# henintsoa98/srsRAN_4G

Hardware: AMD Instinct MI355X
Metric: turbo-decoded info Mbps + PDSCH subframes/s, 20 MHz 64QAM, 1/2/4/8 GPU (higher is better)
Workload: dtype int16; 1 GPU; tdec all 188 LTE CB sizes x 1024 CBs, 8 half-its, rm_turbo SB layout; cb_sizes=188, parallelism=cb-sharded x1, tdec16=auto

## Files before the change

srsran_4g_amd/csrc/tdec_api.cpp:

```cpp
#include <hip/hip_runtime.h>

#include <cstdio>
#include <cstdlib>
#include <algorithm>
#include <cstring>
#include <map>
#include <tuple>
#include <mutex>
#include <vector>

#include "../../include/srsran_tdec.h"
#include "stage_copy.h"
#include "dev_buf.h"
#include "devkey.h"
#include "tdec_kernel.h"
#include "tdec8bit_kernel.h"

using namespace srsran_amd;

namespace {

const uint16_t kCbSizes[SRSRAN_NOF_TC_CB_SIZES] = {
    40,   48,   56,   64,   72,   80,   88,   96,   104,  112,  120,  128,  136,  144,  152,  160,  168,  176,  184,
    192,  200,  208,  216,  224,  232,  240,  248,  256,  264,  272,  280,  288,  296,  304,  312,  320,  328,  336,
// ... 678 lines not shown
  const uint32_t len = (layout_sb && c->nsb > 1) ? 3 * (long_cb + 32) + 12 : 3 * long_cb + 12;
  if (in_stride < len) {
    return SRSRAN_ERROR_INVALID_INPUTS;
  }
  const int n_end = nof_iterations > 0 ? (int)nof_iterations : 1;
  return enqueue(c, d_input, in_stride, layout_sb, d_output, nof_cb, 0, n_end, nullptr, (hipStream_t)stream);
}

namespace {
constexpr int kPoolStreams = 4;
struct MultiDesc {
  PinBuf<char> h_stage;
  DevBuf<char> d_stage;
  hipEvent_t copied  = nullptr;
  bool       used    = false;
};

struct StreamPool {
  int         device = -1;
  hipStream_t s[kPoolStreams];
  hipEvent_t  done[kPoolStreams];
  hipEvent_t  fork;
  hipEvent_t  large_done;
  MultiDesc   md[6];
};
std::mutex               g_pool_mu;
std::vector<StreamPool*> g_pools;

int multi_mode()
{
  static const int m = [] {
    const char* e = getenv("SRSRAN_AMD_TDEC_MULTI");
    return !e ? 0 : !strcmp(e, "priority") ? 1 : !strcmp(e, "serial") ? 2 : 0;
  }();
  return m;
}

StreamPool* get_pool()
{
  int dev = 0;
  if (hipGetDevice(&dev) != hipSuccess) {
    return nullptr;
  }
  std::lock_guard<std::mutex> lk(g_pool_mu);
  for (auto* p : g_pools) {
    if (p->device == dev) {
      return p;
// ... 16 lines not shown
  }
  for (auto& m : p->md) {
    if (srsran_amd::ring_event_create(&m.copied) != hipSuccess) {
      return nullptr;
    }
  }
  g_pools.push_back(p);
  return p;
}

uint32_t gen_cut()
{
  static const uint32_t c = [] {
    const char* e = getenv("SRSRAN_AMD_TDEC_GEN_CUT");
    return e ? (uint32_t)atoi(e) : 0u;
  }();
  return c;
}

uint32_t tdec_midcut()
{
  static const uint32_t c = [] {
    const char* e = getenv("SRSRAN_AMD_TDEC_MIDCUT");
    return e ? (uint32_t)atoi(e) : 3072u;
  }();
  return c;
}
bool tdec_gate()
{
  static const bool g = [] {
    const char* e = getenv("SRSRAN_AMD_TDEC_GATE");
    return e ? atoi(e) != 0 : true;
  }();
  return g;
}

double launch_cost(uint32_t K, uint32_t ncb)
{
  const int    nsb   = auto_nsb(K);
  const double chain = nsb > 1 ? 3.0 * (K / nsb) + 160.0 : 3.0 * (K + 3);
  const double waves = (double)ncb * 4 * nsb / 64.0;
  return chain * (1.0 + waves / 1024.0);
}
}

int srsran_tdec_gpu_run_multi(uint32_t              nof_groups,
                              const uint32_t*       long_cb,
                              const int16_t* const* d_input,
                              const uint32_t*       in_stride,
                              int                   layout_sb,
                              uint8_t* const*       d_output,
                              const uint32_t*       nof_cb,
                              uint32_t              nof_iterations,
                              void*                 stream)
{
  if (nof_groups == 0) {
    return SRSRAN_SUCCESS;
// ... 13 lines not shown
    }
    const uint32_t len = (layout_sb && cfg[g]->nsb > 1) ? 3 * (long_cb[g] + 32) + 12 : 3 * long_cb[g] + 12;
    if (in_stride[g] < len) {
      return SRSRAN_ERROR_INVALID_INPUTS;
    }
    order[g] = g;
  }
  std::sort(order.begin(), order.end(), [&](uint32_t a, uint32_t b) {
    return launch_cost(long_cb[a], nof_cb[a]) > launch_cost(long_cb[b], nof_cb[b]);
  });
  StreamPool* p = get_pool();
  if (!p) {
    return SRSRAN_ERROR;
  }
  hipStream_t user = (hipStream_t)stream;
  if (hipEventRecord(p->fork, user) != hipSuccess) {
    return SRSRAN_ERROR;
  }
  for (int i = 0; i < kPoolStreams; i++) {
    hipStreamWaitEvent(p->s[i], p->fork, 0);
  }
  const int n_end = nof_iterations > 0 ? (int)nof_iterations : 1;
  int       ret   = SRSRAN_SUCCESS;
  const int      cls_nsb[6] = {16, 16, 16, 8, 1, 1};
  const int      cls_st[6]  = {0, 0, 1, 2, 3, 3};
  const uint32_t midcut     = tdec_midcut();
  bool           gated      = false;
  bool           mid_run    = false;
  for (int ci = 0; ci < 6 && ret == SRSRAN_SUCCESS; ci++) {
    if (ci == 1 && hipEventRecord(p->large_done, p->s[0]) != hipSuccess) {
      ret = SRSRAN_ERROR;
      break;
    }
    gated = ci >= 2 && mid_run && tdec_gate() && multi_mode() != 2;
    std::vector<uint32_t> gs;
    uint32_t              cls_cb = 0;
    for (uint32_t i = 0; i < nof_groups; i++) {
      if (cfg[order[i]]->nsb == cls_nsb[ci] && nof_cb[order[i]] > 0) {
        gs.push_back(order[i]);
        cls_cb += nof_cb[order[i]];
      }
    }
    if (gs.empty()) {
      continue;
    }
    const int kind = cls_nsb[ci] == 1               ? (cls_cb >= tdec1s_min_cb() ? 2 : 0)
                     : !layout_sb                   ? 0
                     : cls_nsb[ci] == 16            ? tdec16_choice(cls_cb)
                                                    : (cls_cb >= tdec8s_min_cb() ? 2 : 0);
    const uint32_t cut = std::max(tdecs_w8_max_k(), tdecs_w8_fused_max_k());
    if (cls_nsb[ci] == 16 && kind == 2) {
      const uint32_t lo = ci == 0 ? std::max(cut, midcut) : ci == 1 ? cut : 0;
      const uint32_t hi = ci == 0 ? UINT32_MAX : ci == 1 ? std::max(cut, midcut) : cut;
      gs.erase(std::remove_if(gs.begin(), gs.end(),
                              [&](uint32_t g) { return !(cfg[g]->proto.K > lo && cfg[g]->proto.K <= hi); }),
               gs.end());
    } else if (ci == 1 || ci == 2) {
      gs.clear();
    } else if (ci >= 4 && kind == 0 && gen_cut() > 0) {
      const bool small = ci == 5;
      gs.erase(std::remove_if(gs.begin(), gs.end(), [&](uint32_t g) { return (cfg[g]->proto.K <= gen_cut()) != small; }),
               gs.end());
    } else if (ci == 5) {
      gs.clear();
    }
    if (gs.empty()) {
      continue;
    }
    mid_run        = mid_run || ci == 1;
    hipStream_t st = p->s[multi_mode() == 2 ? 0 : cls_st[ci]];
    if (gated && st != p->s[0] && hipStreamWaitEvent(st, p->large_done, 0) != hipSuccess) {
      ret = SRSRAN_ERROR;
      break;
    }
    if (gs.size() == 1) {
      const uint32_t g = gs[0];
      ret = enqueue(cfg[g], d_input[g], in_stride[g], layout_sb, d_output[g], nof_cb[g], 0, n_end, nullptr, st);
      continue;
    }
    const int  nsbc = cls_nsb[ci];
    uint32_t   kmax = 0;
    for (uint32_t g : gs) {
      kmax = std::max(kmax, cfg[g]->proto.K);
    }
    const bool w8  = kind == 2 && nsbc > 1 && kmax <= (nsbc == 16 ? cut : tdecs_w8_max_k());
    const int  cpw  = kind == 2   ? (nsbc == 16 ? tdecs16::cpw() : nsbc == 8 ? tdecs8::cpw() : tdecs1::cpw())
                      : kind == 1 ? tdec16_cpw()
                                  : tdec_cpw(nsbc);
    const size_t   n     = gs.size();
    const size_t   abyte = n * sizeof(TdecArgs);
    const size_t   need  = abyte + n * sizeof(uint32_t);
    MultiDesc&     m     = p->md[ci];
    if (m.used) {
      hipEventSynchronize(m.copied);
    }
    if (need > m.h_stage.cap() || need > m.d_stage.cap()) {
      hipStreamSynchronize(st);
      if (!m.h_stage.reserve(2 * need) || !m.d_stage.reserve(2 * need)) {
        return SRSRAN_ERROR;
      }
    }
    TdecArgs* ha    = reinterpret_cast<TdecArgs*>(m.h_stage.get());
    uint32_t* hf    = reinterpret_cast<uint32_t*>(m.h_stage + abyte);
    uint32_t  nblk  = 0;
    size_t    lds   = 0;
    for (size_t k = 0; k < n; k++) {
      const uint32_t g = gs[k];
      const Config*  c = cfg[g];
      TdecArgs       a = c->proto;
      a.in             = d_input[g];
      a.in_stride      = in_stride[g];
      a.layout_sb      = c->nsb > 1 ? layout_sb : 0;
      a.ncb            = nof_cb[g];
      a.n_start        = 0;
      a.n_end          = n_end;
      a.out            = d_output[g];
      a.tfwd           = c->d_tfwd;
      a.trev           = c->d_trev;
      a.tfwd_nat       = c->d_tfwd_nat;
      a.trev_nat       = c->d_trev_nat;
      a.state          = nullptr;
      ha[k]            = a;
      hf[k]            = nblk;
      nblk += (nof_cb[g] + cpw - 1) / cpw;
      lds = std::max(lds, kind == 2   ? (nsbc == 16  ? (w8 ? tdecs16w8::lds_bytes(a) : tdecs16::lds_bytes(a))
                                         : nsbc == 8 ? (w8 ? tdecs8w8::lds_bytes(a) : tdecs8::lds_bytes(a))
                                                     : tdecs1::lds_bytes(a))
                          : kind == 1 ? tdec16_lds_bytes(a)
                                      : tdec_lds_bytes(c->nsb, a.xyw, a.M));
    }
    if (hipMemcpyAsync(m.d_stage, m.h_stage, need, hipMemcpyHostToDevice, st) != hipSuccess) {
      return SRSRAN_ERROR;
    }
    hipEventRecord(m.copied, st);
    m.used = true;
    const TdecArgs* dg = reinterpret_cast<const TdecArgs*>(m.d_stage.get());
    const uint32_t* df = reinterpret_cast<const uint32_t*>(m.d_stage + abyte);
    if ((kind == 2   ? (nsbc == 16  ? (w8 ? tdecs16w8::multi_launch(dg, df, (int)n, nblk, lds, st)
                                          : tdecs16::multi_launch(dg, df, (int)n, nblk, lds, st))
                        : nsbc == 8 ? (w8 ? tdecs8w8::multi_launch(dg, df, (int)n, nblk, lds, st)
                                          : tdecs8::multi_launch(dg, df, (int)n, nblk, lds, st))
                                    : tdecs1::multi_launch(dg, df, (int)n, nblk, lds, st))
         : kind == 1 ? tdec16_multi_launch(dg, df, (int)n, nblk, lds, st)
                     : tdec_multi_launch(cls_nsb[ci], dg, df, (int)n, nblk, lds, st)) != hipSuccess) {
      ret = SRSRAN_ERROR;
    }
  }
  for (int i = 0; i < kPoolStreams; i++) {
    hipEventRecord(p->done[i], p->s[i]);
    hipStreamWaitEvent(user, p->done[i], 0);
  }
  return ret;
}

#ifdef TDECS_STAMPS
int srsran_tdec_gpu_debug_set_stamps(void* d_buf)
{
  using namespace srsran_amd;
  return tdecs16::set_stamps(d_buf) == hipSuccess && tdecs8::set_stamps(d_buf) == hipSuccess &&
                 tdecs16w8::set_stamps(d_buf) == hipSuccess && tdecs8w8::set_stamps(d_buf) == hipSuccess
             ? SRSRAN_SUCCESS
             : SRSRAN_ERROR;
// ... 117 lines not shown
```

srsran_4g_amd/csrc/tdec_kernel.h:

```cpp
#ifndef SRSRAN_AMD_TDEC_KERNEL_H
#define SRSRAN_AMD_TDEC_KERNEL_H
#include <hip/hip_runtime.h>
#include <stddef.h>
#include <stdint.h>

namespace srsran_amd {

static constexpr int TDEC_W       = 32;
static constexpr int TDEC_OVERLAP = 40;

struct TdecCb {
  const short*   in;
  const uint8_t* skip;
  uint32_t       slot;
  uint32_t       crc_a;
};
static constexpr uint32_t TDEC_PAD_SLOT = 0xffffffffu;
static constexpr uint64_t TDEC_PAIR_SPAN = ((uint64_t)1 << 31) - ((uint64_t)1 << 16);
static constexpr uint32_t TDEC_GROUP     = 8;

struct TdecArgs {
  const short*    in;
  uint32_t        in_stride;
  int             layout_sb;
// ... 33 lines not shown
bool       tdec16_eligible(int nsb, const TdecArgs& a);
bool       tdec16_pays(uint32_t ncb);
void       tdec16_set_min_cb(uint32_t n);
uint32_t   tdec16_min_cb();
hipError_t tdec16_launch(const TdecArgs& a, hipStream_t stream);
hipError_t tdec16_multi_launch(const TdecArgs* d_groups, const uint32_t* d_first, int ngroups, uint32_t nblocks,
                               size_t lds, hipStream_t stream);
size_t     tdec16_lds_bytes(const TdecArgs& a);
int        tdec16_cpw();
#define SRSRAN_TDECS_API(ns)                                                                               \
  namespace ns {                                                                                           \
  hipError_t launch(const TdecArgs& a, hipStream_t stream);                                                \
  hipError_t multi_launch(const TdecArgs* d_groups, const uint32_t* d_first, int ngroups, uint32_t nblocks, \
                          size_t lds, hipStream_t stream);                                                 \
  size_t     lds_bytes(const TdecArgs& a);                                                                 \
  int        cpw();                                                                                        \
  }
SRSRAN_TDECS_API(tdecs16)
SRSRAN_TDECS_API(tdecs8)
SRSRAN_TDECS_API(tdecs16w8)
SRSRAN_TDECS_API(tdecs8w8)
SRSRAN_TDECS_API(tdecs1)
#undef SRSRAN_TDECS_API
#ifdef TDECS_STAMPS
namespace tdecs16 { hipError_t set_stamps(void* d_buf); }
namespace tdecs8 { hipError_t set_stamps(void* d_buf); }
namespace tdecs16w8 { hipError_t set_stamps(void* d_buf); }
namespace tdecs8w8 { hipError_t set_stamps(void* d_buf); }
#endif
bool       tdec8s_eligible(int nsb, const TdecArgs& a);
bool       tdec1s_eligible(int nsb, const TdecArgs& a);
void       tdecs_set_w8_max_k(uint32_t k);
void       tdecs_set_w8_fused_max_k(uint32_t k);
uint32_t   tdecs_w8_fused_max_k();
uint32_t   tdecs_w8_max_k();
void       tdec8s_set_min_cb(uint32_t n);
uint32_t   tdec8s_min_cb();
void       tdec1s_set_min_cb(uint32_t n);
uint32_t   tdec1s_min_cb();
void       tdec16s_set_min_cb(uint32_t n);
uint32_t   tdec16s_min_cb();
int        tdec16_choice(uint32_t ncb);
size_t     tdec_lds_bytes(int nsb, int xyw, int M);
void crc24_xpow_table(uint32_t poly, uint32_t* out, int nm);

int tdec_sch_enqueue(uint32_t      K,
// ... 18 lines not shown
```

srsran_4g_amd/csrc/tdecs_kernel.hip:

```cpp
#include <hip/hip_runtime.h>
#include <stdint.h>

#include "crc24_dev.h"
#include "stage_timing.h"
#include "tdec_kernel.h"

#ifndef TDECS_NSB
#define TDECS_NSB 16
#endif
#ifndef TDECS_W
#define TDECS_W 16
#endif
#if TDECS_NSB == 16 && TDECS_W == 16
#define TDECS_NS tdecs16
#define TDECS_K(n) tdec16s_##n
#define TDECS_NAME "tdec16s_"
#elif TDECS_NSB == 8 && TDECS_W == 16
#define TDECS_NS tdecs8
#define TDECS_K(n) tdec8s_##n
#define TDECS_NAME "tdec8s_"
#elif TDECS_NSB == 16 && TDECS_W == 8
#define TDECS_NS tdecs16w8
#define TDECS_K(n) tdec16sw8_##n
#define TDECS_NAME "tdec16sw8_"
#elif TDECS_NSB == 8 && TDECS_W == 8
#define TDECS_NS tdecs8w8
#define TDECS_K(n) tdec8sw8_##n
#define TDECS_NAME "tdec8sw8_"
#else
#error "TDECS_NSB must be 16 or 8, TDECS_W 16 or 8"
#endif

namespace srsran_amd {
namespace TDECS_NS {
namespace {

typedef short v2s __attribute__((ext_vector_type(2)));

constexpr int   W    = TDECS_W;
constexpr int   OVL  = TDEC_OVERLAP;
constexpr int   NTR  = (OVL + W - 1) / W;
constexpr int   NSB  = TDECS_NSB;
constexpr short NEG  = -10000;
constexpr int   CPWG = 64 / NSB;
constexpr int   ROWB = 2 * NSB;

#ifdef TDECS_STAMPS
__device__ unsigned long long* g_stamps = nullptr;
#define TDECS_STAMP(k)                                                                               \
  do {                                                                                               \
    if ((threadIdx.x & 63) == 0 && g_stamps && (k) < 64) {                                          \
      g_stamps[((size_t)blockIdx.x * (blockDim.x >> 6) + (threadIdx.x >> 6)) * 64 + (k)] = clock64(); \
    }                                                                                                \
  } while (0)
// ... 91 lines not shown
#pragma unroll
  for (int t = 2; t >= 0; t--) {
    const short x = xt[t], y = yt[t], xy = (short)(x + y);
    short       n[8];
    n[0] = max(o[0], (short)(o[4] + xy));
    n[1] = max((short)(o[0] + xy), o[4]);
    n[2] = max((short)(o[1] + x), (short)(o[5] + y));
    n[3] = max((short)(o[1] + y), (short)(o[5] + x));
    n[4] = max((short)(o[2] + y), (short)(o[6] + x));
    n[5] = max((short)(o[2] + x), (short)(o[6] + y));
    n[6] = max((short)(o[3] + xy), o[7]);
    n[7] = max(o[3], (short)(o[7] + xy));
#pragma unroll
    for (int i = 0; i < 8; i++) {
      o[i] = n[i];
    }
  }
  return St{v2s{o[0], o[4]}, v2s{o[7], o[3]}, v2s{o[2], o[6]}, v2s{o[5], o[1]}};
}

struct Geo {
  int s_dw, ck_dw, bits_dw, cb_dw;
};
__host__ __device__ __forceinline__ Geo geo(int K, int Ls, int M, bool slot)
{
  Geo g;
  g.s_dw    = (NSB * Ls + 1) / 2;
  g.ck_dw   = M * NSB * 4;
  g.bits_dw = slot ? (NSB * Ls + 31) / 32 + 1 : (K / 8 + 3) / 4;
  g.cb_dw   = g.s_dw + g.ck_dw + g.bits_dw + 2;
  return g;
}

struct Raw {
  uint32_t a[W];
  uint16_t slot[W];
  uint32_t b[W];
};

typedef short __attribute__((address_space(3)))* lshort;
typedef __amdgpu_buffer_rsrc_t                   rsrc_t;
__device__ __forceinline__ uint32_t ldb(rsrc_t r, uint32_t voff, uint32_t soff, int imm)
{
  return __builtin_amdgcn_raw_buffer_load_b16(r, voff + imm, soff, 0);
}
__device__ __forceinline__ rsrc_t make_rsrc(const void* p, uint32_t bytes)
{
  const size_t   u  = (size_t)p;
  const uint32_t lo = __builtin_amdgcn_readfirstlane((uint32_t)u);
  const uint32_t hi = __builtin_amdgcn_readfirstlane((uint32_t)(u >> 32));
  return __builtin_amdgcn_make_buffer_rsrc((void*)(((size_t)hi << 32) | lo), 0,
                                           (int)__builtin_amdgcn_readfirstlane(bytes), 0x00020000);
}

struct Lane {
  int       s, K, L, Ls, M, KP;
  uint32_t  magicLs;
  rsrc_t    rin;
  uint32_t  voff;
  rsrc_t    rtf;
  lshort    S;
  lshort    Ssb;
  uint4*    CK;
  uint32_t* BITS;
};

__device__ __forceinline__ void ck_put(const Lane& c, int m, const St& p)
{
  c.CK[m * NSB + c.s] = make_uint4(v2u(p.a), v2u(p.b), v2u(p.c), v2u(p.d));
}
__device__ __forceinline__ St ck_get(const Lane& c, int m)
{
  const uint4 v = c.CK[m * NSB + c.s];
  return St{u2v(v.x), u2v(v.y), u2v(v.z), u2v(v.w)};
}

template <bool D2>
__device__ __forceinline__ void issue(const Lane& c, Raw& r, int t0)
{
  const uint32_t soff = (uint32_t)ROWB * (uint32_t)t0;
  const uint32_t poff = soff + (D2 ? 4u : 2u) * (uint32_t)c.KP;
#ifdef TDECS_FAKELOAD
#pragma unroll
  for (int i = 0; i < W; i++) {
    r.a[i]    = (soff + i) & 0xff;
    r.slot[i] = (uint16_t)((c.s * 37 + t0 + i) & 511);
    r.b[i] = (poff + 3 * i) & 0xff;
  }
#else
#pragma unroll
  for (int i = 0; i < W; i++) {
    if (D2) {
      r.slot[i] = (uint16_t)ldb(c.rtf, 2u * (uint32_t)c.s, soff, ROWB * i);
    } else {
      r.a[i] = ldb(c.rin, c.voff, soff, ROWB * i);
    }
    r.b[i] = ldb(c.rin, c.voff, poff, ROWB * i);
  }
#endif
}

__device__ __forceinline__ uint32_t pin(uint32_t v)
{
  asm volatile("" : "+v"(v));
  return v;
}

__device__ __forceinline__ void set_nat(const Lane& c, int n, short o)
{
  atomicOr(&c.BITS[n >> 5], (uint32_t)(o > 0) << (((n >> 3) & 3) * 8 + 7 - (n & 7)));
}

template <bool D2, int BITS>
__device__ __forceinline__ uint32_t emit(const Lane& c, int k, short o, uint32_t aux, uint32_t xw)
{
  if (D2) {
    const lshort p = (lshort)(size_t)aux;
    *p             = (short)(o - (short)(xw & 0xffffu));
    if (BITS == 2) {
      const uint32_t slot = (uint32_t)(p - c.S);
      atomicOr(&c.BITS[slot >> 5], (uint32_t)(o > 0) << (slot & 31));
    } else if (BITS == 1) {
      const int slot = (int)(p - c.S);
      const int sb   = (int)__umulhi((uint32_t)slot, c.magicLs);
      set_nat(c, slot - sb * (c.Ls - c.L), o);
    }
    return 0;
  }
// ... 10 lines not shown
    const uint32_t pos = (uint32_t)(c.s * c.Ls + t0);
    const uint64_t v   = (uint64_t)wbits << (pos & 31);
    atomicOr(&c.BITS[pos >> 5], (uint32_t)v);
    if ((uint32_t)(v >> 32)) {
      atomicOr(&c.BITS[(pos >> 5) + 1], (uint32_t)(v >> 32));
    }
  }
}

__device__ __forceinline__ uint32_t nat_byte(const uint32_t* bits, int L, int Ls, uint32_t magicL, int b)
{
  const int      n0  = 8 * b;
  const int      j   = (int)__umulhi((uint32_t)n0, magicL);
  const int      cnt = (j + 1) * L - n0;
  const uint32_t s0  = (uint32_t)(n0 + j * (Ls - L));
  const uint64_t v   = (uint64_t)bits[s0 >> 5] | (uint64_t)bits[(s0 >> 5) + 1] << 32;
  uint32_t       x   = (uint32_t)(v >> (s0 & 31)) & 0x1ffu;
  if (cnt < 8) {
    x = (x & ((1u << cnt) - 1u)) | ((x >> (cnt + Ls - L)) << cnt);
  }
  return __builtin_bitreverse32(x & 0xffu) >> 24;
}

template <bool D2, int BITS, bool FULL>
__device__ __forceinline__ St alpha_llr_window(const Lane& c, St P, int t0, St Pb, const uint32_t* xw,
                                               const uint32_t* aux)
{
  const int L  = c.L;
  const int cc = FULL ? t0 + W : L;
  const int ic = cc - t0 - 1;
  St        bw[W];
#pragma unroll
  for (int i = W - 1; i >= 0; i--) {
    if (FULL ? i == W - 1 : i == ic) {
      bw[i] = Pb;
      if (cc < L && norm_at(cc)) Pb = norm(Pb);
    } else if (FULL || i < ic) {
      Pb    = step<true>(Pb, xw[i + 1]);
      bw[i] = Pb;
      if (FULL ? (i & 1) : norm_at(t0 + 1 + i)) Pb = norm(Pb);
    }
  }
  uint32_t wbits = 0;
#pragma unroll
  for (int i = 0; i < W; i++) {
    if (FULL || t0 + i < L) {
      const Cand  cd = cand(P, bm(xw[i]));
      const short o  = llr(cd, bw[i]);
      P              = next<false>(cd);
      if ((i & 1) == 0) P = norm(P);
      wbits |= emit<D2, BITS>(c, t0 + i, o, aux[i], xw[i]) << i;
    }
  }
  if (BITS == 2 && !D2) {
    flush_bits(c, t0, wbits);
  }
  return P;
}

template <bool FULL>
__device__ __forceinline__ St beta_window(const Lane& c, St P, int t0, bool store, St& Bst, const uint32_t* xw)
{
#pragma unroll
  for (int i = W - 1; i >= 0; i--) {
    if (FULL || t0 + i < c.L) {
      P = step<true>(P, xw[i]);
      if (i == 0) {
        Bst = P;
        if (store) {
          ck_put(c, t0 / W - 1, P);
        }
      }
      if ((i & 1) == 0) P = norm(P);
    }
  }
  return P;
}

template <int IMM>
__device__ __forceinline__ void wait_for()
{
  __builtin_amdgcn_sched_barrier(0);
  __builtin_amdgcn_s_waitcnt(IMM);
  __builtin_amdgcn_sched_barrier(0);
}
__device__ __forceinline__ void wait_vm0() { wait_for<0x0f70>(); }
__device__ __forceinline__ void wait_lgkm0() { wait_for<0xc07f>(); }
__device__ __forceinline__ void wait_all0() { wait_for<0x0070>(); }

__device__ __forceinline__ uint32_t slot_addr(lshort S, uint16_t slot)
{
  uint32_t a;
  asm("v_mad_u32_u16 %0, %1, 2, %2" : "=v"(a) : "v"(__builtin_bit_cast(_Float16, slot)), "v"((uint32_t)(size_t)S));
// ... 47 lines not shown
      if (!LAST) {
        issue<D2>(c, g, tnext);
      }
      wait_lgkm0();
#pragma unroll
      for (int i = 0; i < W; i++) {
        xw[i] = pin(v2u(pack((uint16_t)d[i], pb[i])));
      }
    } else {
      wait_all0();
#pragma unroll
      for (int i = 0; i < W; i++) {
        xw[i]  = pin(v2u(padd(pack(g.a[i], g.b[i]), u2v(dv[i]))));
        aux[i] = dv[i];
      }
      __builtin_amdgcn_sched_barrier(0);
      if (!LAST) {
        load(c, tnext);
      }
    }
  }
};

template <bool D2, int BITS>
__device__ __forceinline__ void map16s(const Lane& cin, int wave, int st0)
{
  (void)st0;
  Lane c = cin;
  asm volatile("" : "+v"(c.s));
  asm volatile("" : "+v"(c.voff));
  {
    uint32_t ssb = (uint32_t)(size_t)c.Ssb;
    asm volatile("" : "+v"(ssb));
    c.Ssb = (lshort)(size_t)ssb;
  }
  const int L     = c.L;
  const int Mfull = L / W;
  const int Ma    = (L + W - 1) / W;
  const int h     = max(1, min((L + 2 * W - 1) / (2 * W), L / W));
  Pipe<D2>  pp;
  uint32_t  xw[W];
  uint32_t  aux[W];
  if (wave == 0) {
    pp.start(c, L - OVL);
    St P = neg_state();
    TDECS_STAMP(st0);
#pragma unroll
    for (int w = 0; w < NTR; w++) {
      pp.next(c, w < NTR - 1 ? L - OVL + W * (w + 1) : 0, xw, aux);
#pragma unroll
      for (int i = 0; i < (W < OVL - w * W ? W : OVL - w * W); i++) {
        P = step<false>(P, xw[i]);
        if (norm_at(w * W + i)) P = norm(P);
      }
      pp.taken(c);
    }
    TDECS_STAMP(st0 + 1);
    {
      St q;
      q.a = u2v((uint32_t)__shfl_up((int)v2u(P.a), 1, NSB));
      q.b = u2v((uint32_t)__shfl_up((int)v2u(P.b), 1, NSB));
      q.c = u2v((uint32_t)__shfl_up((int)v2u(P.c), 1, NSB));
      q.d = u2v((uint32_t)__shfl_up((int)v2u(P.d), 1, NSB));
      P   = c.s == 0 ? alpha_known() : q;
    }
#pragma unroll 1
    for (int ma = 0; ma < h; ma++) {
      const int t0 = ma * W;
      pp.next(c, t0 + W, xw, aux);
      ck_put(c, ma, P);
#pragma unroll
      for (int i = 0; i < W; i++) {
        P = step<false>(P, xw[i]);
        if (nrm(t0, i)) P = norm(P);
      }
      pp.taken(c);
    }
    TDECS_STAMP(st0 + 2);
    __syncthreads();
    TDECS_STAMP(st0 + 3);
    const int tlast = (Ma - 1) * W;
#pragma unroll 1
    for (int ma = h; ma < Mfull; ma++) {
      pp.next(c, min(ma * W + W, tlast), xw, aux);
      P = alpha_llr_window<D2, BITS, true>(c, P, ma * W, ck_get(c, ma), xw, aux);
      pp.taken(c);
    }
    if (Ma > Mfull) {
      pp.template next<true>(c, 0, xw, aux);
      alpha_llr_window<D2, BITS, false>(c, P, Mfull * W, ck_get(c, Mfull), xw, aux);
    }
    TDECS_STAMP(st0 + 4);
  } else {
    pp.start(c, (NTR - 1) * W);
    St P = neg_state();
    TDECS_STAMP(st0);
#pragma unroll
    for (int w = 0; w < NTR; w++) {
      const int t0 = (NTR - 1 - w) * W;
      pp.next(c, w < NTR - 1 ? t0 - W : (Ma - 1) * W, xw, aux);
#pragma unroll
      for (int i = (W < OVL - t0 ? W : OVL - t0) - 1; i >= 0; i--) {
        P = step<true>(P, xw[i]);
        if (norm_at(t0 + i)) P = norm(P);
      }
      pp.taken(c);
    }
    TDECS_STAMP(st0 + 1);
    {
      St q;
      q.a = u2v((uint32_t)__shfl_down((int)v2u(P.a), 1, NSB));
      q.b = u2v((uint32_t)__shfl_down((int)v2u(P.b), 1, NSB));
      q.c = u2v((uint32_t)__shfl_down((int)v2u(P.c), 1, NSB));
      q.d = u2v((uint32_t)__shfl_down((int)v2u(P.d), 1, NSB));
      if (c.s == NSB - 1) {
        const int tail = 6 * c.KP + (D2 ? 12 : 0);
        short     xt[3], yt[3];
#pragma unroll
        for (int t = 0; t < 3; t++) {
          xt[t] = (short)ldb(c.rin, c.voff - 2 * c.s, tail, 4 * t);
          yt[t] = (short)ldb(c.rin, c.voff - 2 * c.s, tail, 4 * t + 2);
        }
        P = trellis(xt, yt);
      } else {
        P = q;
      }
    }
    const int mtop = Ma - 1;
    ck_put(c, mtop, P);
    St Bst = P;
    if (Ma > Mfull) {
      pp.next(c, (mtop - 1) * W, xw, aux);
      P = beta_window<false>(c, P, mtop * W, mtop > h, Bst, xw);
      pp.taken(c);
    }
#pragma unroll 1
    for (int mb = Mfull - 1; mb >= h; mb--) {
      pp.next(c, mb * W - W, xw, aux);
      P = beta_window<true>(c, P, mb * W, mb > h, Bst, xw);
      pp.taken(c);
    }
    TDECS_STAMP(st0 + 2);
    __syncthreads();
    TDECS_STAMP(st0 + 3);
#pragma unroll 1
    for (int mb = h - 1; mb >= 0; mb--) {
      const int t0 = mb * W;
      pp.next(c, max(t0 - W, 0), xw, aux);
      St Pa = ck_get(c, mb);
      St aw[W];
#pragma unroll
      for (int i = 0; i < W; i++) {
        aw[i] = Pa;
        if (i < W - 1) {
          Pa = step<false>(Pa, xw[i]);
          if (nrm(t0, i)) Pa = norm(Pa);
        }
      }
      uint32_t wbits = 0;
#pragma unroll
      for (int i = W - 1; i >= 0; i--) {
        const short o = llr(cand(aw[i], bm(xw[i])), Bst);
        P             = step<true>(P, xw[i]);
        Bst           = P;
        if (nrm(t0, i)) P = norm(P);
        wbits |= emit<D2, BITS>(c, t0 + i, o, aux[i], xw[i]) << i;
      }
      if (BITS == 2 && !D2) {
        flush_bits(c, t0, wbits);
      }
      pp.taken(c);
    }
    TDECS_STAMP(st0 + 4);
  }
}

}

template <bool ES>
__device__ __forceinline__ void body(const TdecArgs& a, int bid)
{
  constexpr int NT = 128;
  extern __shared__ __attribute__((aligned(16))) uint32_t smem[];
  const int lane = threadIdx.x & 63;
  const int wave = threadIdx.x >> 6;
  const int cbw  = lane / NSB;
  const int s    = lane % NSB;
  const int t2   = wave * NSB + s;
  const int K    = (int)a.K;
  const int L    = (int)a.L;
  const int Ls   = (int)a.Ls;
  const int M    = (L + W - 1) / W;
  const Geo g    = geo(K, Ls, M, ES);
  const int cb   = bid * CPWG + cbw;
  const int cbl  = cb < (int)a.ncb ? cb : (int)a.ncb - 1;
  const bool live = cb < (int)a.ncb && (!ES || a.cbs[cbl].slot != TDEC_PAD_SLOT);
  bool done      = ES && (!live || *a.cbs[cbl].skip);

  uint32_t* base = smem + cbw * g.cb_dw;
  Lane      c;
  c.s       = s;
  c.K       = K;
  c.L       = L;
  c.Ls      = Ls;
  c.M       = M;
  c.KP      = K + 32;
  c.magicLs = a.magicLs;
  const uint32_t magicL = 0xffffffffu / (uint32_t)L + 1u;
  const int cb0 = bid * CPWG;
  size_t    in_lane, in_lo = SIZE_MAX, in_hi = 0;
#pragma unroll
  for (int i = 0; i < CPWG; i++) {
    const int    j = min(cb0 + i, (int)a.ncb - 1);
    const size_t p = ES ? (size_t)a.cbs[j].in : (size_t)(a.in + (size_t)j * a.in_stride);
    in_lo          = min(in_lo, p);
    in_hi          = max(in_hi, p);
  }
  in_lane                 = ES ? (size_t)a.cbs[cbl].in : (size_t)(a.in + (size_t)cbl * a.in_stride);
  const uint32_t cb_bytes = (uint32_t)(3 * c.KP + 12) * 2;
  c.rin  = make_rsrc((const void*)in_lo, (uint32_t)(in_hi - in_lo) + cb_bytes);
  c.voff = (uint32_t)(in_lane - in_lo) + 2 * c.s;
  c.rtf  = make_rsrc(a.tfwd, 2u * (uint32_t)K);
  c.S    = (lshort)(short*)base;
  c.Ssb  = c.S + c.s * Ls;
  c.CK   = reinterpret_cast<uint4*>(base + g.s_dw);
  c.BITS = base + g.s_dw + g.ck_dw;
  uint32_t* RED = c.BITS + g.bits_dw;

  if constexpr (ES) {
    if (live && done && t2 == 0) {
      const uint32_t slot = a.cbs[cbl].slot;
      a.noi_out[slot]     = 0;
      a.crc_ok[slot]      = 1;
    }
  }
  for (int i = threadIdx.x; i < CPWG * g.s_dw; i += NT) {
    smem[(i / g.s_dw) * g.cb_dw + i % g.s_dw] = 0u;
  }
  const int h_end = (ES && __syncthreads_or(!done) == 0) ? 0 : a.n_end;
#ifdef TDECS_STAMPS
  int passed_at = 0, ran = 0;
#endif

#pragma unroll 1
  for (int hi = 0; hi < h_end; hi++) {
    const bool crc_now = ES && hi + 1 >= a.min_iters;
    for (int i = threadIdx.x; i < CPWG * g.bits_dw; i += NT) {
      smem[(i / g.bits_dw) * g.cb_dw + g.s_dw + g.ck_dw + i % g.bits_dw] = 0u;
    }
    __syncthreads();
    const bool    bits = ES ? crc_now : hi + 1 == h_end;
    constexpr int BM   = ES ? 2 : 1;
    if (hi & 1) {
      if (bits) {
        map16s<true, BM>(c, wave, 5 * hi);
      } else {
        map16s<true, 0>(c, wave, 5 * hi);
      }
    } else {
      if (bits) {
        map16s<false, BM>(c, wave, 5 * hi);
      } else {
        map16s<false, 0>(c, wave, 5 * hi);
      }
    }
    __syncthreads();

    if constexpr (ES) {
      if (crc_now) {
        const int      nbytes = K / 8;
        const int      bpt    = (nbytes + 2 * NSB - 1) / (2 * NSB);
        const int      b0     = t2 * bpt;
        const int      b1     = min(b0 + bpt, nbytes);
        const bool     crc_a  = a.cbs[cbl].crc_a;
        const uint32_t poly   = crc_a ? LTE_CRC24A : LTE_CRC24B;
        uint32_t       crc    = 0;
#pragma unroll 1
        for (int b = b0; b < b1; b++) {
          crc = crc24_byte(crc, nat_byte(c.BITS, L, Ls, magicL, b), poly);
        }
        uint32_t part = b0 < nbytes ? clmul_mod24(crc, (crc_a ? a.xpow_a : a.xpow_b)[nbytes - b1], poly) : 0;
#pragma unroll
        for (int off = 1; off < NSB; off <<= 1) {
          part ^= (uint32_t)__shfl_xor((int)part, off, 64);
        }
        if (s == 0) {
// ... 36 lines not shown
    }
  }
#endif

  if (live && !done && h_end > 0) {
    const int      cbm   = ES ? (int)a.cbs[cbl].slot : cbl;
    uint8_t*       out   = a.out + (size_t)cbm * (ES ? a.out_stride : K / 8);
    for (int b = t2; b < K / 8; b += 2 * NSB) {
      out[b] = ES ? (uint8_t)nat_byte(c.BITS, L, Ls, magicL, b) : reinterpret_cast<const uint8_t*>(c.BITS)[b];
    }
    if (ES && t2 == 0) {
      a.noi_out[cbm] = (uint8_t)a.n_end;
      a.crc_ok[cbm]  = 0;
    }
  }
}

template <bool ES>
__global__ __launch_bounds__(128, 1) void TDECS_K(kernel)(TdecArgs a)
{
  body<ES>(a, blockIdx.x);
}

__global__ __launch_bounds__(128, 1) void TDECS_K(multi_kernel)(const TdecArgs* __restrict__ groups,
                                                            const uint32_t* __restrict__ first, int ngroups)
{
  if constexpr (NSB == 16 && W == 16) {
    __builtin_amdgcn_s_setprio(2);
  }
  const uint32_t b  = blockIdx.x;
  int            lo = 0, hi = ngroups - 1;
  while (lo < hi) {
    const int mid = (lo + hi + 1) >> 1;
    if (first[mid] <= b) {
      lo = mid;
    } else {
      hi = mid - 1;
    }
  }
  const TdecArgs a = groups[lo];
  body<false>(a, (int)(b - first[lo]));
}

size_t lds_bytes(const TdecArgs& a)
{
  const Geo g = geo((int)a.K, (int)a.Ls, (int)((a.L + W - 1) / W), a.cbs != nullptr);
  return (size_t)CPWG * g.cb_dw * 4;
}

int cpw() { return CPWG; }

hipError_t launch(const TdecArgs& a, hipStream_t stream)
{
  StageScope timing_scope(ST_TDEC, stream);
  const int    grid = (a.ncb + CPWG - 1) / CPWG;
  const size_t lds  = lds_bytes(a);
  tdec_set_last_kernel(a.cbs ? TDECS_NAME "kernel<true>" : TDECS_NAME "kernel<false>");
  if (a.cbs) {
    hipLaunchKernelGGL((TDECS_K(kernel)<true>), dim3(grid), dim3(128), lds, stream, a);
  } else {
    hipLaunchKernelGGL((TDECS_K(kernel)<false>), dim3(grid), dim3(128), lds, stream, a);
  }
  return hipGetLastError();
}

hipError_t multi_launch(const TdecArgs* d_groups, const uint32_t* d_first, int ngroups, uint32_t nblocks, size_t lds,
                        hipStream_t stream)
{
  StageScope timing_scope(ST_TDEC, stream);
  if (ngroups == 0 || nblocks == 0) {
    return hipSuccess;
  }
  tdec_set_last_kernel(TDECS_NAME "multi_kernel");
  hipLaunchKernelGGL(TDECS_K(multi_kernel), dim3(nblocks), dim3(128), lds, stream, d_groups, d_first, ngroups);
  return hipGetLastError();
}

#ifdef TDECS_STAMPS
hipError_t set_stamps(void* d_buf)
{
  unsigned long long* p = (unsigned long long*)d_buf;
  return hipMemcpyToSymbol(HIP_SYMBOL(g_stamps), &p, sizeof(p));
}
#endif

}
}
```

Measured before the change: 35450 Mbps.

## Move NSB16 turbo-decoder checkpoints from LDS to global buffer to raise occupancy

```diff
diff --git a/srsran_4g_amd/csrc/tdec_api.cpp b/srsran_4g_amd/csrc/tdec_api.cpp
--- a/srsran_4g_amd/csrc/tdec_api.cpp
+++ b/srsran_4g_amd/csrc/tdec_api.cpp
@@ -724,7 +724,9 @@
   hipEvent_t  done[kPoolStreams];
   hipEvent_t  fork;
   hipEvent_t  large_done;
-  MultiDesc   md[6];
+  MultiDesc   md[7];
+  DevBuf<uint8_t>       d_ck;
+  std::map<size_t, int> wg_per_cu;
 };
 std::mutex               g_pool_mu;
 std::vector<StreamPool*> g_pools;
@@ -787,7 +789,7 @@
 {
   static const uint32_t c = [] {
     const char* e = getenv("SRSRAN_AMD_TDEC_MIDCUT");
-    return e ? (uint32_t)atoi(e) : 3072u;
+    return e ? (uint32_t)atoi(e) : 2048u;
   }();
   return c;
 }
@@ -798,6 +800,15 @@
     return e ? atoi(e) != 0 : true;
   }();
   return g;
+}
+
+int fused16_wg_per_cu(StreamPool* p, size_t lds)
+{
+  auto it = p->wg_per_cu.find(lds);
+  if (it == p->wg_per_cu.end()) {
+    it = p->wg_per_cu.emplace(lds, tdecs16::multi_wg_per_cu(lds)).first;
+  }
+  return it->second;
 }
 
 double launch_cost(uint32_t K, uint32_t ncb)
@@ -857,17 +868,36 @@
   }
   const int n_end = nof_iterations > 0 ? (int)nof_iterations : 1;
   int       ret   = SRSRAN_SUCCESS;
-  const int      cls_nsb[6] = {16, 16, 16, 8, 1, 1};
-  const int      cls_st[6]  = {0, 0, 1, 2, 3, 3};
+  const int      cls_nsb[7] = {16, 16, 16, 16, 8, 1, 1};
+  const int      cls_st[7]  = {0, 0, 0, 1, 2, 3, 3};
   const uint32_t midcut     = tdec_midcut();
+  const uint32_t cut        = std::max(tdecs_w8_max_k(), tdecs_w8_fused_max_k());
   bool           gated      = false;
   bool           mid_run    = false;
-  for (int ci = 0; ci < 6 && ret == SRSRAN_SUCCESS; ci++) {
-    if (ci == 1 && hipEventRecord(p->large_done, p->s[0]) != hipSuccess) {
+  uint64_t ck_need = 0, ck_used = 0;
+  const Config* top16 = nullptr;
+  for (uint32_t g = 0; g < nof_groups && layout_sb; g++) {
+    if (cfg[g]->nsb == 16 && cfg[g]->proto.K > cut && nof_cb[g] > 0) {
+      TdecArgs a = cfg[g]->proto;
+      a.ncb      = nof_cb[g];
+      ck_need += tdecs16::multi_ck_bytes(a);
+      top16 = top16 && top16->proto.K > a.K ? top16 : cfg[g];
+    }
+  }
+  if (ck_need > p->d_ck.cap()) {
+    hipStreamSynchronize(p->s[0]);
+    if (!p->d_ck.reserve(ck_need)) {
+      return SRSRAN_ERROR;
+    }
+  }
+  auto residency = [&](const Config* c) { return fused16_wg_per_cu(p, tdecs16::multi_lds_bytes(c->proto)); };
+  const int top_res = top16 ? residency(top16) : 0;
+  for (int ci = 0; ci < 7 && ret == SRSRAN_SUCCESS; ci++) {
+    if (ci == 2 && hipEventRecord(p->large_done, p->s[0]) != hipSuccess) {
       ret = SRSRAN_ERROR;
       break;
     }
-    gated = ci >= 2 && mid_run && tdec_gate() && multi_mode() != 2;
+    gated = ci >= 3 && mid_run && tdec_gate() && multi_mode() != 2;
     std::vector<uint32_t> gs;
     uint32_t              cls_cb = 0;
     for (uint32_t i = 0; i < nof_groups; i++) {
@@ -883,26 +913,28 @@
                      : !layout_sb                   ? 0
                      : cls_nsb[ci] == 16            ? tdec16_choice(cls_cb)
                                                     : (cls_cb >= tdec8s_min_cb() ? 2 : 0);
-    const uint32_t cut = std::max(tdecs_w8_max_k(), tdecs_w8_fused_max_k());
     if (cls_nsb[ci] == 16 && kind == 2) {
-      const uint32_t lo = ci == 0 ? std::max(cut, midcut) : ci == 1 ? cut : 0;
-      const uint32_t hi = ci == 0 ? UINT32_MAX : ci == 1 ? std::max(cut, midcut) : cut;
+      const uint32_t lo = ci <= 1 ? std::max(cut, midcut) : ci == 2 ? cut : 0;
+      const uint32_t hi = ci <= 1 ? UINT32_MAX : ci == 2 ? std::max(cut, midcut) : cut;
       gs.erase(std::remove_if(gs.begin(), gs.end(),
-                              [&](uint32_t g) { return !(cfg[g]->proto.K > lo && cfg[g]->proto.K <= hi); }),
+                              [&](uint32_t g) {
+                                const uint32_t K = cfg[g]->proto.K;
+                                return !(K > lo && K <= hi) || (ci <= 1 && (residency(cfg[g]) == top_res) != (ci == 0));
+                              }),
                gs.end());
-    } else if (ci == 1 || ci == 2) {
+    } else if (ci >= 1 && ci <= 3) {
       gs.clear();
-    } else if (ci >= 4 && kind == 0 && gen_cut() > 0) {
-      const bool small = ci == 5;
+    } else if (ci >= 5 && kind == 0 && gen_cut() > 0) {
+      const bool small = ci == 6;
       gs.erase(std::remove_if(gs.begin(), gs.end(), [&](uint32_t g) { return (cfg[g]->proto.K <= gen_cut()) != small; }),
                gs.end());
-    } else if (ci == 5) {
+    } else if (ci == 6) {
       gs.clear();
     }
     if (gs.empty()) {
       continue;
     }
-    mid_run        = mid_run || ci == 1;
+    mid_run        = mid_run || ci == 2;
     hipStream_t st = p->s[multi_mode() == 2 ? 0 : cls_st[ci]];
     if (gated && st != p->s[0] && hipStreamWaitEvent(st, p->large_done, 0) != hipSuccess) {
       ret = SRSRAN_ERROR;
@@ -919,12 +951,14 @@
       kmax = std::max(kmax, cfg[g]->proto.K);
     }
     const bool w8  = kind == 2 && nsbc > 1 && kmax <= (nsbc == 16 ? cut : tdecs_w8_max_k());
+    const bool gck = kind == 2 && nsbc == 16 && !w8;
     const int  cpw  = kind == 2   ? (nsbc == 16 ? tdecs16::cpw() : nsbc == 8 ? tdecs8::cpw() : tdecs1::cpw())
                       : kind == 1 ? tdec16_cpw()
                                   : tdec_cpw(nsbc);
     const size_t   n     = gs.size();
     const size_t   abyte = n * sizeof(TdecArgs);
-    const size_t   need  = abyte + n * sizeof(uint32_t);
+    const size_t   kbyte = n * sizeof(uint64_t);
+    const size_t   need  = abyte + kbyte + n * sizeof(uint32_t);
     MultiDesc&     m     = p->md[ci];
     if (m.used) {
       hipEventSynchronize(m.copied);
@@ -936,7 +970,8 @@
       }
     }
     TdecArgs* ha    = reinterpret_cast<TdecArgs*>(m.h_stage.get());
-    uint32_t* hf    = reinterpret_cast<uint32_t*>(m.h_stage + abyte);
+    uint64_t* hk    = reinterpret_cast<uint64_t*>(m.h_stage + abyte);
+    uint32_t* hf    = reinterpret_cast<uint32_t*>(m.h_stage + abyte + kbyte);
     uint32_t  nblk  = 0;
     size_t    lds   = 0;
     for (size_t k = 0; k < n; k++) {
@@ -955,10 +990,14 @@
       a.tfwd_nat       = c->d_tfwd_nat;
       a.trev_nat       = c->d_trev_nat;
       a.state          = nullptr;
+      hk[k] = ck_used;
+      if (gck) {
+        ck_used += tdecs16::multi_ck_bytes(a);
+      }
       ha[k]            = a;
       hf[k]            = nblk;
       nblk += (nof_cb[g] + cpw - 1) / cpw;
-      lds = std::max(lds, kind == 2   ? (nsbc == 16  ? (w8 ? tdecs16w8::lds_bytes(a) : tdecs16::lds_bytes(a))
+      lds = std::max(lds, kind == 2   ? (nsbc == 16  ? (w8 ? tdecs16w8::lds_bytes(a) : tdecs16::multi_lds_bytes(a))
                                          : nsbc == 8 ? (w8 ? tdecs8w8::lds_bytes(a) : tdecs8::lds_bytes(a))
                                                      : tdecs1::lds_bytes(a))
                           : kind == 1 ? tdec16_lds_bytes(a)
@@ -970,9 +1009,11 @@
     hipEventRecord(m.copied, st);
     m.used = true;
     const TdecArgs* dg = reinterpret_cast<const TdecArgs*>(m.d_stage.get());
-    const uint32_t* df = reinterpret_cast<const uint32_t*>(m.d_stage + abyte);
+    const uint64_t* dk = reinterpret_cast<const uint64_t*>(m.d_stage + abyte);
+    const uint32_t* df = reinterpret_cast<const uint32_t*>(m.d_stage + abyte + kbyte);
     if ((kind == 2   ? (nsbc == 16  ? (w8 ? tdecs16w8::multi_launch(dg, df, (int)n, nblk, lds, st)
-                                          : tdecs16::multi_launch(dg, df, (int)n, nblk, lds, st))
+                                          : tdecs16::multi_launch_ck(dg, df, dk, (int)n, nblk, lds, p->d_ck.get(),
+                                                                     p->d_ck.cap(), st))
                         : nsbc == 8 ? (w8 ? tdecs8w8::multi_launch(dg, df, (int)n, nblk, lds, st)
                                           : tdecs8::multi_launch(dg, df, (int)n, nblk, lds, st))
                                     : tdecs1::multi_launch(dg, df, (int)n, nblk, lds, st))
diff --git a/srsran_4g_amd/csrc/tdec_kernel.h b/srsran_4g_amd/csrc/tdec_kernel.h
--- a/srsran_4g_amd/csrc/tdec_kernel.h
+++ b/srsran_4g_amd/csrc/tdec_kernel.h
@@ -79,6 +79,13 @@
 SRSRAN_TDECS_API(tdecs8w8)
 SRSRAN_TDECS_API(tdecs1)
 #undef SRSRAN_TDECS_API
+namespace tdecs16 {
+hipError_t multi_launch_ck(const TdecArgs* d_groups, const uint32_t* d_first, const uint64_t* d_ck_off, int ngroups,
+                           uint32_t nblocks, size_t lds, uint8_t* d_ck, uint64_t ck_bytes, hipStream_t stream);
+size_t     multi_lds_bytes(const TdecArgs& a);
+uint64_t   multi_ck_bytes(const TdecArgs& a);
+int        multi_wg_per_cu(size_t lds);
+}
 #ifdef TDECS_STAMPS
 namespace tdecs16 { hipError_t set_stamps(void* d_buf); }
 namespace tdecs8 { hipError_t set_stamps(void* d_buf); }
diff --git a/srsran_4g_amd/csrc/tdecs_ck_geo.h b/srsran_4g_amd/csrc/tdecs_ck_geo.h
--- /dev/null
+++ b/srsran_4g_amd/csrc/tdecs_ck_geo.h
@@ -0,0 +1,33 @@
+#ifndef SRSRAN_AMD_TDECS_CK_GEO_H
+#define SRSRAN_AMD_TDECS_CK_GEO_H
+#include <stddef.h>
+#include <stdint.h>
+
+#if defined(__HIPCC__) || defined(__CUDACC__)
+#define TDECS_CK_HD __host__ __device__
+#else
+#define TDECS_CK_HD
+#endif
+
+namespace srsran_amd {
+
+static constexpr uint32_t TDECS_CK_W     = 16;
+static constexpr uint32_t TDECS_CK_LANES = 64;
+static constexpr uint32_t TDECS_CK_STATE = 16;
+static constexpr uint32_t TDECS_CK_ROW   = TDECS_CK_LANES * TDECS_CK_STATE;
+
+TDECS_CK_HD inline uint32_t tdecs_ck_windows(uint32_t L) { return (L + TDECS_CK_W - 1) / TDECS_CK_W; }
+TDECS_CK_HD inline uint32_t tdecs_ck_wg_bytes(uint32_t L) { return tdecs_ck_windows(L) * TDECS_CK_ROW; }
+TDECS_CK_HD inline uint64_t tdecs_ck_group_bytes(uint32_t L, uint32_t nwg) { return (uint64_t)nwg * tdecs_ck_wg_bytes(L); }
+TDECS_CK_HD inline uint64_t tdecs_ck_wg_off(uint32_t L, uint32_t wg) { return (uint64_t)wg * tdecs_ck_wg_bytes(L); }
+TDECS_CK_HD inline uint32_t tdecs_ck_wg_avail(uint32_t L, uint32_t wg, uint64_t group_bytes)
+{
+  const uint64_t off = tdecs_ck_wg_off(L, wg);
+  const uint64_t len = tdecs_ck_wg_bytes(L);
+  return off >= group_bytes ? 0u : (uint32_t)(group_bytes - off < len ? group_bytes - off : len);
+}
+TDECS_CK_HD inline uint32_t tdecs_ck_row(int m) { return (uint32_t)m * TDECS_CK_ROW; }
+TDECS_CK_HD inline uint32_t tdecs_ck_lane(uint32_t lane) { return lane * TDECS_CK_STATE; }
+
+}
+#endif
diff --git a/srsran_4g_amd/csrc/tdecs_kernel.hip b/srsran_4g_amd/csrc/tdecs_kernel.hip
--- a/srsran_4g_amd/csrc/tdecs_kernel.hip
+++ b/srsran_4g_amd/csrc/tdecs_kernel.hip
@@ -4,6 +4,7 @@
 #include "crc24_dev.h"
 #include "stage_timing.h"
 #include "tdec_kernel.h"
+#include "tdecs_ck_geo.h"
 
 #ifndef TDECS_NSB
 #define TDECS_NSB 16
@@ -30,6 +31,11 @@
 #else
 #error "TDECS_NSB must be 16 or 8, TDECS_W 16 or 8"
 #endif
+#if TDECS_NSB == 16 && TDECS_W == 16
+#define TDECS_GCK 1
+#else
+#define TDECS_GCK 0
+#endif
 
 namespace srsran_amd {
 namespace TDECS_NS {
@@ -167,11 +173,11 @@
 struct Geo {
   int s_dw, ck_dw, bits_dw, cb_dw;
 };
-__host__ __device__ __forceinline__ Geo geo(int K, int Ls, int M, bool slot)
+__host__ __device__ __forceinline__ Geo geo(int K, int Ls, int M, bool slot, bool gck = false)
 {
   Geo g;
   g.s_dw    = (NSB * Ls + 1) / 2;
-  g.ck_dw   = M * NSB * 4;
+  g.ck_dw   = gck ? 0 : M * NSB * 4;
   g.bits_dw = slot ? (NSB * Ls + 31) / 32 + 1 : (K / 8 + 3) / 4;
   g.cb_dw   = g.s_dw + g.ck_dw + g.bits_dw + 2;
   return g;
@@ -207,15 +213,29 @@
   lshort    S;
   lshort    Ssb;
   uint4*    CK;
+  rsrc_t    rck;
+  uint32_t  ckv;
   uint32_t* BITS;
 };
 
+typedef uint32_t v4u __attribute__((ext_vector_type(4)));
+template <bool GCK>
 __device__ __forceinline__ void ck_put(const Lane& c, int m, const St& p)
 {
-  c.CK[m * NSB + c.s] = make_uint4(v2u(p.a), v2u(p.b), v2u(p.c), v2u(p.d));
-}
+  if (GCK) {
+    const v4u v = {v2u(p.a), v2u(p.b), v2u(p.c), v2u(p.d)};
+    __builtin_amdgcn_raw_buffer_store_b128(v, c.rck, c.ckv, tdecs_ck_row(m), 0);
+  } else {
+    c.CK[m * NSB + c.s] = make_uint4(v2u(p.a), v2u(p.b), v2u(p.c), v2u(p.d));
+  }
+}
+template <bool GCK>
 __device__ __forceinline__ St ck_get(const Lane& c, int m)
 {
+  if (GCK) {
+    const v4u v = __builtin_amdgcn_raw_buffer_load_b128(c.rck, c.ckv, tdecs_ck_row(m), 0);
+    return St{u2v(v.x), u2v(v.y), u2v(v.z), u2v(v.w)};
+  }
   const uint4 v = c.CK[m * NSB + c.s];
   return St{u2v(v.x), u2v(v.y), u2v(v.z), u2v(v.w)};
 }
@@ -249,6 +269,10 @@
 {
   asm volatile("" : "+v"(v));
   return v;
+}
+[[maybe_unused]] __device__ __forceinline__ St pin(const St& p)
+{
+  return St{u2v(pin(v2u(p.a))), u2v(pin(v2u(p.b))), u2v(pin(v2u(p.c))), u2v(pin(v2u(p.d)))};
 }
 
 __device__ __forceinline__ void set_nat(const Lane& c, int n, short o)
@@ -305,7 +329,7 @@
   return __builtin_bitreverse32(x & 0xffu) >> 24;
 }
 
-template <bool D2, int BITS, bool FULL>
+template <bool D2, int BITS, bool FULL, bool GCK = false>
 __device__ __forceinline__ St alpha_llr_window(const Lane& c, St P, int t0, St Pb, const uint32_t* xw,
                                                const uint32_t* aux)
 {
@@ -328,7 +352,7 @@
 #pragma unroll
   for (int i = 0; i < W; i++) {
     if (FULL || t0 + i < L) {
-      const Cand  cd = cand(P, bm(xw[i]));
+      const Cand  cd = cand(P, bm(GCK ? pin(xw[i]) : xw[i]));
       const short o  = llr(cd, bw[i]);
       P              = next<false>(cd);
       if ((i & 1) == 0) P = norm(P);
@@ -341,7 +365,7 @@
   return P;
 }
 
-template <bool FULL>
+template <bool FULL, bool GCK = false>
 __device__ __forceinline__ St beta_window(const Lane& c, St P, int t0, bool store, St& Bst, const uint32_t* xw)
 {
 #pragma unroll
@@ -351,7 +375,7 @@
       if (i == 0) {
         Bst = P;
         if (store) {
-          ck_put(c, t0 / W - 1, P);
+          ck_put<GCK>(c, t0 / W - 1, P);
         }
       }
       if ((i & 1) == 0) P = norm(P);
@@ -445,7 +469,19 @@
   }
 };
 
-template <bool D2, int BITS>
+template <bool GCK>
+__device__ __forceinline__ void phase_barrier()
+{
+  if (GCK) {
+    __builtin_amdgcn_fence(__ATOMIC_RELEASE, "workgroup");
+  }
+  __syncthreads();
+  if (GCK) {
+    __builtin_amdgcn_fence(__ATOMIC_ACQUIRE, "workgroup");
+  }
+}
+
+template <bool D2, int BITS, bool GCK = false>
 __device__ __forceinline__ void map16s(const Lane& cin, int wave, int st0)
 {
   (void)st0;
@@ -491,7 +527,7 @@
     for (int ma = 0; ma < h; ma++) {
       const int t0 = ma * W;
       pp.next(c, t0 + W, xw, aux);
-      ck_put(c, ma, P);
+      ck_put<GCK>(c, ma, P);
 #pragma unroll
       for (int i = 0; i < W; i++) {
         P = step<false>(P, xw[i]);
@@ -500,18 +536,29 @@
       pp.taken(c);
     }
     TDECS_STAMP(st0 + 2);
-    __syncthreads();
+    phase_barrier<GCK>();
     TDECS_STAMP(st0 + 3);
     const int tlast = (Ma - 1) * W;
+    St        ckc;
+    if (GCK) {
+      ckc = ck_get<true>(c, h);
+    }
 #pragma unroll 1
     for (int ma = h; ma < Mfull; ma++) {
       pp.next(c, min(ma * W + W, tlast), xw, aux);
-      P = alpha_llr_window<D2, BITS, true>(c, P, ma * W, ck_get(c, ma), xw, aux);
+      St ckn;
+      if (GCK) {
+        ckn = ck_get<true>(c, min(ma + 1, Ma - 1));
+      }
+      P = alpha_llr_window<D2, BITS, true, GCK>(c, P, ma * W, GCK ? ckc : ck_get<false>(c, ma), xw, aux);
       pp.taken(c);
+      if (GCK) {
+        ckc = ckn;
+      }
     }
     if (Ma > Mfull) {
       pp.template next<true>(c, 0, xw, aux);
-      alpha_llr_window<D2, BITS, false>(c, P, Mfull * W, ck_get(c, Mfull), xw, aux);
+      alpha_llr_window<D2, BITS, false, GCK>(c, P, Mfull * W, GCK ? ckc : ck_get<false>(c, Mfull), xw, aux);
     }
     TDECS_STAMP(st0 + 4);
   } else {
@@ -550,27 +597,34 @@
       }
     }
     const int mtop = Ma - 1;
-    ck_put(c, mtop, P);
+    ck_put<GCK>(c, mtop, P);
     St Bst = P;
     if (Ma > Mfull) {
       pp.next(c, (mtop - 1) * W, xw, aux);
-      P = beta_window<false>(c, P, mtop * W, mtop > h, Bst, xw);
+      P = beta_window<false, GCK>(c, P, mtop * W, mtop > h, Bst, xw);
       pp.taken(c);
     }
 #pragma unroll 1
     for (int mb = Mfull - 1; mb >= h; mb--) {
       pp.next(c, mb * W - W, xw, aux);
-      P = beta_window<true>(c, P, mb * W, mb > h, Bst, xw);
+      P = beta_window<true, GCK>(c, P, mb * W, mb > h, Bst, xw);
       pp.taken(c);
     }
     TDECS_STAMP(st0 + 2);
-    __syncthreads();
+    phase_barrier<GCK>();
     TDECS_STAMP(st0 + 3);
+    St ckc;
+    if (GCK) {
+      ckc = ck_get<true>(c, h - 1);
+    }
 #pragma unroll 1
     for (int mb = h - 1; mb >= 0; mb--) {
       const int t0 = mb * W;
       pp.next(c, max(t0 - W, 0), xw, aux);
-      St Pa = ck_get(c, mb);
+      St Pa = GCK ? ckc : ck_get<false>(c, mb);
+      if (GCK) {
+        ckc = ck_get<true>(c, max(mb - 1, 0));
+      }
       St aw[W];
 #pragma unroll
       for (int i = 0; i < W; i++) {
@@ -583,7 +637,12 @@
       uint32_t wbits = 0;
 #pragma unroll
       for (int i = W - 1; i >= 0; i--) {
-        const short o = llr(cand(aw[i], bm(xw[i])), Bst);
+        short o;
+        if constexpr (GCK) {
+          o = llr(cand(pin(aw[i]), bm(pin(xw[i]))), Bst);
+        } else {
+          o = llr(cand(aw[i], bm(xw[i])), Bst);
+        }
         P             = step<true>(P, xw[i]);
         Bst           = P;
         if (nrm(t0, i)) P = norm(P);
@@ -600,8 +659,8 @@
 
 }
 
-template <bool ES>
-__device__ __forceinline__ void body(const TdecArgs& a, int bid)
+template <bool ES, bool GCK = false>
+__device__ __forceinline__ void body(const TdecArgs& a, int bid, uint8_t* ck = nullptr, uint64_t ck_bytes = 0)
 {
   constexpr int NT = 128;
   extern __shared__ __attribute__((aligned(16))) uint32_t smem[];
@@ -614,7 +673,7 @@
   const int L    = (int)a.L;
   const int Ls   = (int)a.Ls;
   const int M    = (L + W - 1) / W;
-  const Geo g    = geo(K, Ls, M, ES);
+  const Geo g    = geo(K, Ls, M, ES, GCK);
   const int cb   = bid * CPWG + cbw;
   const int cbl  = cb < (int)a.ncb ? cb : (int)a.ncb - 1;
   const bool live = cb < (int)a.ncb && (!ES || a.cbs[cbl].slot != TDEC_PAD_SLOT);
@@ -648,6 +707,10 @@
   c.Ssb  = c.S + c.s * Ls;
   c.CK   = reinterpret_cast<uint4*>(base + g.s_dw);
   c.BITS = base + g.s_dw + g.ck_dw;
+  if constexpr (GCK) {
+    c.rck = make_rsrc(ck + tdecs_ck_wg_off((uint32_t)L, (uint32_t)bid), tdecs_ck_wg_avail((uint32_t)L, (uint32_t)bid, ck_bytes));
+    c.ckv = tdecs_ck_lane((uint32_t)lane);
+  }
   uint32_t* RED = c.BITS + g.bits_dw;
 
   if constexpr (ES) {
@@ -676,15 +739,15 @@
     constexpr int BM   = ES ? 2 : 1;
     if (hi & 1) {
       if (bits) {
-        map16s<true, BM>(c, wave, 5 * hi);
+        map16s<true, BM, GCK>(c, wave, 5 * hi);
       } else {
-        map16s<true, 0>(c, wave, 5 * hi);
+        map16s<true, 0, GCK>(c, wave, 5 * hi);
       }
     } else {
       if (bits) {
-        map16s<false, BM>(c, wave, 5 * hi);
+        map16s<false, BM, GCK>(c, wave, 5 * hi);
       } else {
-        map16s<false, 0>(c, wave, 5 * hi);
+        map16s<false, 0, GCK>(c, wave, 5 * hi);
       }
     }
     __syncthreads();
@@ -767,8 +830,13 @@
   body<ES>(a, blockIdx.x);
 }
 
-__global__ __launch_bounds__(128, 1) void TDECS_K(multi_kernel)(const TdecArgs* __restrict__ groups,
-                                                            const uint32_t* __restrict__ first, int ngroups)
+__global__ __launch_bounds__(128, TDECS_GCK ? 2 : 1) void TDECS_K(multi_kernel)(const TdecArgs* __restrict__ groups,
+                                                            const uint32_t* __restrict__ first, int ngroups
+#if TDECS_GCK
+                                                            , const uint64_t* __restrict__ ck_off, uint8_t* ck,
+                                                            uint64_t ck_bytes
+#endif
+)
 {
   if constexpr (NSB == 16 && W == 16) {
     __builtin_amdgcn_s_setprio(2);
@@ -784,7 +852,13 @@
     }
   }
   const TdecArgs a = groups[lo];
+#if TDECS_GCK
+  const uint64_t off  = ck_off[lo];
+  const uint64_t part = tdecs_ck_group_bytes(a.L, (a.ncb + CPWG - 1) / CPWG);
+  body<false, true>(a, (int)(b - first[lo]), ck + off, off >= ck_bytes ? 0 : min(part, ck_bytes - off));
+#else
   body<false>(a, (int)(b - first[lo]));
+#endif
 }
 
 size_t lds_bytes(const TdecArgs& a)
@@ -792,6 +866,23 @@
   const Geo g = geo((int)a.K, (int)a.Ls, (int)((a.L + W - 1) / W), a.cbs != nullptr);
   return (size_t)CPWG * g.cb_dw * 4;
 }
+
+#if TDECS_GCK
+size_t multi_lds_bytes(const TdecArgs& a)
+{
+  const Geo g = geo((int)a.K, (int)a.Ls, (int)((a.L + W - 1) / W), false, true);
+  return (size_t)CPWG * g.cb_dw * 4;
+}
+uint64_t multi_ck_bytes(const TdecArgs& a)
+{
+  return tdecs_ck_group_bytes(a.L, (a.ncb + CPWG - 1) / CPWG);
+}
+int multi_wg_per_cu(size_t lds)
+{
+  int n = 0;
+  return hipOccupancyMaxActiveBlocksPerMultiprocessor(&n, TDECS_K(multi_kernel), 128, lds) == hipSuccess ? n : 0;
+}
+#endif
 
 int cpw() { return CPWG; }
 
@@ -816,10 +907,29 @@
   if (ngroups == 0 || nblocks == 0) {
     return hipSuccess;
   }
+#if TDECS_GCK
+  return hipErrorInvalidValue;
+#else
   tdec_set_last_kernel(TDECS_NAME "multi_kernel");
   hipLaunchKernelGGL(TDECS_K(multi_kernel), dim3(nblocks), dim3(128), lds, stream, d_groups, d_first, ngroups);
   return hipGetLastError();
-}
+#endif
+}
+
+#if TDECS_GCK
+hipError_t multi_launch_ck(const TdecArgs* d_groups, const uint32_t* d_first, const uint64_t* d_ck_off, int ngroups,
+                           uint32_t nblocks, size_t lds, uint8_t* d_ck, uint64_t ck_bytes, hipStream_t stream)
+{
+  StageScope timing_scope(ST_TDEC, stream);
+  if (ngroups == 0 || nblocks == 0) {
+    return hipSuccess;
+  }
+  tdec_set_last_kernel(TDECS_NAME "multi_kernel");
+  hipLaunchKernelGGL(TDECS_K(multi_kernel), dim3(nblocks), dim3(128), lds, stream, d_groups, d_first, ngroups, d_ck_off,
+                     d_ck, ck_bytes);
+  return hipGetLastError();
+}
+#endif
 
 #ifdef TDECS_STAMPS
 hipError_t set_stamps(void* d_buf)
```

After: 36420 Mbps (median of 6 runs). +2.7%, better.
